# sidward14/gan-lab

Hardware: AMD Instinct MI355X
Metric: images/sec (G+D step), StyleGAN 1024^2 bs32/GPU (higher is better)
Workload: dtype f32; 1 GPU; StyleGAN res_samples=1024 FFHQ-shaped synthetic, bs=32/GPU fp32, nonsaturating + R1(lambda=10) + drift, stabilised phase, 1 D-iter + 1 G-iter; global_batch=32, per_gpu_batch=32, parallelism=single

## Files before the change

### gan_lab_amd/_lib.py

```python
import ctypes
import os
import subprocess

import torch

_HERE = os.path.dirname(os.path.abspath(__file__))
CSRC = os.path.join(_HERE, 'csrc')
SO_PATH = os.path.join(CSRC, os.path.basename(os.environ.get('GANLAB_HIP_LIB', '') or 'libganlab_hip.so'))

_c_int, _c_ll, _c_f, _c_p, _c_sz, _c_u64 = (ctypes.c_int, ctypes.c_longlong, ctypes.c_float, ctypes.c_void_p,
                                             ctypes.c_size_t, ctypes.c_uint64)

ACT_NONE, ACT_LRELU = 0, 1
PACK_FWD, PACK_DGRAD = 0, 1


class ConvGeom(ctypes.Structure):
    _fields_ = [('N', _c_int), ('Cin', _c_int), ('Hin', _c_int), ('Win', _c_int),
                ('Cout', _c_int), ('ks', _c_int), ('pad', _c_int), ('up', _c_int), ('pool', _c_int)]


_GP = ctypes.POINTER(ConvGeom)


# ... 41 lines not shown
    'ganlab_conv_splitk_plan': (_c_int, [_GP, _c_int]),
    'ganlab_conv_fwd_splitk_f32': (_c_int, [_c_p, _c_p, _c_p, _c_p, _GP, _c_f, _c_int, _c_f, _c_p, _c_sz, _c_p]),
    'ganlab_conv_dgrad_splitk_f32': (_c_int, [_c_p, _c_p, _c_p, _GP, _c_p, _c_sz, _c_p]),
    'ganlab_conv_dgrad_mask_supported': (_c_int, [_GP]),
    'ganlab_conv_dgrad_mask_f32': (_c_int, [_c_p, _c_p, _c_p, _c_p, _GP, _c_f, _c_p]),
    'ganlab_conv_act_bwd_fused_supported': (_c_int, [_GP]),
    'ganlab_conv_dgrad_act_f32': (_c_int, [_c_p, _c_p, _c_p, _c_p, _GP, _c_f, _c_p]),
    'ganlab_conv_fwd_mask_f32': (_c_int, [_c_p, _c_p, _c_p, _c_p, _GP, _c_f, _c_p]),
    'ganlab_conv_wgrad_act_f32': (_c_int, [_c_p, _c_p, _c_p, _c_p, _c_p, _GP, _c_f, _c_f, _c_f, _c_p, _c_sz, _c_p]),
    'ganlab_conv_wgrad_workspace': (_c_sz, [_GP]),
    'ganlab_conv_wgrad_f32': (_c_int, [_c_p, _c_p, _c_p, _GP, _c_f, _c_p, _c_sz, _c_p]),
    'ganlab_conv_s2_supported': (_c_int, [_GP]),
    'ganlab_conv_s2_pack_f32': (_c_ll, [_c_p, _c_p, _c_int, _c_int, _c_int, _c_int, _c_f, _c_p]),
    'ganlab_conv_s2_fwd_f32': (_c_int, [_c_p, _c_p, _c_p, _c_p, _GP, _c_f, _c_int, _c_f, _c_p]),
    'ganlab_conv_s2_dgrad_f32': (_c_int, [_c_p, _c_p, _c_p, _GP, _c_p]),
    'ganlab_conv_s2_wgrad_workspace': (_c_sz, [_GP]),
    'ganlab_conv_s2_wgrad_f32': (_c_int, [_c_p, _c_p, _c_p, _GP, _c_f, _c_p, _c_sz, _c_p]),
    'ganlab_conv_bf16_supported': (_c_int, [_GP]),
    'ganlab_conv_pack_bf16': (_c_ll, [_c_p, _c_p, _c_int, _c_int, _c_int, _c_f, _c_p]),
    'ganlab_conv_fwd_bf16': (_c_int, [_c_p, _c_p, _c_p, _c_p, _GP, _c_f, _c_int, _c_f, _c_p]),
    'ganlab_conv_dgrad_bf16': (_c_int, [_c_p, _c_p, _c_p, _GP, _c_p]),
    'ganlab_conv_bf16_splitk_plan': (_c_int, [_GP, _c_int]),
    'ganlab_conv_fwd_bf16_splitk': (_c_int, [_c_p, _c_p, _c_p, _c_p, _GP, _c_f, _c_int, _c_f, _c_p, _c_sz, _c_p]),
    'ganlab_conv_dgrad_bf16_splitk': (_c_int, [_c_p, _c_p, _c_p, _GP, _c_p, _c_sz, _c_p]),
    'ganlab_conv_wgrad_bf16_workspace': (_c_sz, [_GP]),
    'ganlab_conv_wgrad_bf16': (_c_int, [_c_p, _c_p, _c_p, _GP, _c_f, _c_p, _c_sz, _c_p]),
    'ganlab_conv_x3_supported': (_c_int, [_GP, _c_int]),
    'ganlab_conv_x3_pack': (_c_ll, [_c_p, _c_p, _c_int, _c_int, _c_int, _c_f, _c_p]),
    'ganlab_conv_fwd_x3': (_c_int, [_c_p, _c_p, _c_p, _c_p, _GP, _c_f, _c_int, _c_f, _c_p]),
    'ganlab_conv_dgrad_x3': (_c_int, [_c_p, _c_p, _c_p, _GP, _c_p]),
# ... 296 lines not shown
```

### gan_lab_amd/csrc/common.h

```cpp
#pragma once
#include <hip/hip_runtime.h>
#include <stdint.h>

#include "../../include/ganlab_hip.h"

typedef float f32x4 __attribute__((ext_vector_type(4)));

static thread_local int gl_launch_status = GANLAB_OK;
extern thread_local const void* gl_last_kernel_fn;
extern thread_local unsigned gl_last_grid;
#define GL_LAUNCH_RING 16
extern thread_local const void* gl_ring_fn[GL_LAUNCH_RING];
extern thread_local unsigned gl_ring_grid[GL_LAUNCH_RING];
extern thread_local unsigned long long gl_launch_count;
#define GL_LAUNCH(k, grid, ...)                                                  \
  do {                                                                           \
    (void)hipGetLastError();                                                     \
    const dim3 gl_grid_ = (grid);                                                \
    gl_last_kernel_fn = reinterpret_cast<const void*>(k);                        \
    gl_last_grid = gl_grid_.x * gl_grid_.y * gl_grid_.z;                         \
    gl_ring_fn[gl_launch_count % GL_LAUNCH_RING] = gl_last_kernel_fn;            \
    gl_ring_grid[gl_launch_count % GL_LAUNCH_RING] = gl_last_grid;               \
    ++gl_launch_count;                                                           \
    hipLaunchKernelGGL(k, gl_grid_, __VA_ARGS__);                                \
// ... 131 lines not shown
          const int kgq = ty * 2 + tx;
          base[((0 * 4 + kgq) * 128 + px * 64 + col) * 8 + j] = p.h;
          base[((1 * 4 + kgq) * 128 + px * 64 + col) * 8 + j] = p.m;
          base[((2 * 4 + kgq) * 128 + px * 64 + col) * 8 + j] = p.l;
        }
}

__device__ __forceinline__ float gl_comb_s2(int up, int a, int k) {
  if (up) {
    const int lo = (a == 0) ? 2 : (a == 1 ? 1 : 0), hi = (a == 0) ? 2 : (a == 1 ? 2 : (a == 2 ? 1 : 0));
    return (k >= lo && k <= hi) ? 1.f : 0.f;
  }
  const int lo = (a <= 1) ? 0 : (a == 2 ? 1 : 2), hi = (a == 0) ? 0 : (a == 1 ? 1 : 2);
  return (k >= lo && k <= hi) ? 0.5f : 0.f;
}
__device__ __forceinline__ void gl_x3_down_pack_position(const float* __restrict__ w9, int up, float scale, __bf16* __restrict__ out,
                                                         int CI, int ci, int co) {
  const int nsteps = CI / 8 * 4;
  const int ct = co >> 7, col = co & 127, q = ci >> 3, j = ci & 7;
  float k9[9];
#pragma unroll
  for (int t = 0; t < 9; ++t) k9[t] = w9[t];
#pragma unroll
  for (int a = 0; a < 4; ++a)
#pragma unroll
    for (int b = 0; b < 4; ++b) {
      float v = 0.f;
#pragma unroll
      for (int ky = 0; ky < 3; ++ky)
#pragma unroll
// ... 13 lines not shown

bool gl_wgrad_roll_supported(int N, int Cin, int Cout, int H, int W, int ks, int pad, int up, const void* x,
                             const void* gy);
int gl_wgrad_roll_slots(int N, int Cin, int Cout, int H, int W);
int gl_wgrad_roll_launch(const float* x, const float* gy, float* part, int N, int Cin, int Cout, int H, int W,
                         hipStream_t st, const float* aff_s = nullptr, const float* aff_t = nullptr);
bool gl_wgrad_s2_roll_supported(int N, int Cl, int Ch, int Hl, int Wl, const void* low, const void* high);
int gl_wgrad_s2_roll_slots(int N, int Cl, int Ch, int Hl, int Wl);
int gl_wgrad_s2_roll_launch(const float* low, const float* high, float* part, int N, int Cl, int Ch, int Hl, int Wl,
                            hipStream_t st, const float* aff_s = nullptr, const float* aff_t = nullptr);

bool gl_s2_roll_supported(int is_T, int N, int Cin, int Cout, int Hl, int Wl, const void* x, const void* y);
int gl_s2_roll_launch(int is_T, const float* x, const float* wp, const float* bias, float* y, int N, int Cin, int Cout,
                      int Hl, int Wl, int Cin_p, int Cout_p, float bias_scale, int act, float slope, hipStream_t st,
                      const float* aff_s = nullptr, const float* aff_t = nullptr);

bool gl_roll_blur_supported(int N, int Cin, int Cout, int H, int W, const void* x, const void* y);
int gl_roll_blur_launch(const float* x, const float* wp, const float* bias, float* y, void* bits, int N, int Cin, int Cout,
                        int H, int W, int Cin_p, int Cout_p, float bias_scale, float slope, hipStream_t st, int blur, int act);
```

### gan_lab_amd/csrc/conv_s2.hip

```cpp
#include "common.h"

#include <stdlib.h>

namespace {
typedef unsigned int u32x4 __attribute__((ext_vector_type(4)));

constexpr int round_up_c(int v, int m) { return (v + m - 1) / m * m; }
constexpr int ceil_div_c(int a, int b) { return (a + b - 1) / b; }
constexpr int pad_mod32(int v, int r) { return v + ((r - (v % 32)) + 32) % 32; }
inline int ceil_div(int a, int b) { return (a + b - 1) / b; }
inline bool aligned16(const void* p) { return (reinterpret_cast<uintptr_t>(p) & 15) == 0; }

__device__ __constant__ const int kDY[4] = {-1, 0, 0, 1};
__device__ __constant__ const int kPY[4] = {1, 0, 1, 0};
constexpr int cDY(int a) { return a == 0 ? -1 : (a == 3 ? 1 : 0); }
constexpr int cPY(int a) { return (a == 0 || a == 2) ? 1 : 0; }

__device__ __forceinline__ float comb(int up, int a, int k) {
  if (up) {
    const int lo = (a == 0) ? 2 : (a == 1 ? 1 : 0), hi = (a == 0) ? 2 : (a == 1 ? 2 : (a == 2 ? 1 : 0));
    return (k >= lo && k <= hi) ? 1.f : 0.f;
  }
  const int lo = (a <= 1) ? 0 : (a == 2 ? 1 : 2), hi = (a == 0) ? 0 : (a == 1 ? 1 : 2);
  return (k >= lo && k <= hi) ? 0.5f : 0.f;
// ... 5 lines not shown
  for (long long e = blockIdx.x * (long long)blockDim.x + threadIdx.x; e < total;
       e += (long long)gridDim.x * blockDim.x) {
    const int col = (int)(e % cols_p);
    const long long t = e / cols_p;
    const int row = (int)(t % rows_p), tap = (int)(t / rows_p);
    float v = 0.f;
    if (row < rows && col < cols) {
      const int co = transpose ? row : col, ci = transpose ? col : row;
      const int a = tap >> 2, b = tap & 3;
      const float* ws = w + ((long long)co * Cin + ci) * 9;
#pragma unroll
      for (int ky = 0; ky < 3; ++ky)
#pragma unroll
        for (int kx = 0; kx < 3; ++kx) v += comb(up, a, ky) * comb(up, b, kx) * ws[ky * 3 + kx];
      v *= scale;
    }
    out[e] = v;
  }
}

struct S2Args {
  const float* x;
  const float* wp;
  const float* bias;
  float* y;
  int N, Cin, Cout;
  int Hl, Wl;
  int Cin_p, Cout_p;
  int tiles_x, tiles_y, tiles_co;
  float bias_scale, slope;
// ... 1037 lines not shown
}

long long ganlab_conv_s2_pack_f32(const float* w, float* out, int Cout, int Cin, int up, int transpose, float scale,
                                  void* stream) {
  if (Cout <= 0 || Cin <= 0) return GANLAB_EINVAL;
  const int rows = transpose ? Cout : Cin, cols = transpose ? Cin : Cout;
  const int rows_p = round_up_c(rows, 16), cols_p = round_up_c(cols, 64);
  const long long total = 16LL * rows_p * cols_p;
  if (!out) return total;
  if (!w) return GANLAB_EINVAL;
  long long blocks = (total + 255) / 256;
  if (blocks > 4096) blocks = 4096;
  GL_LAUNCH(pack_s2_kernel, dim3((unsigned)blocks), dim3(256), 0, gl_stream(stream), w, out, Cout, Cin, rows, cols,
            rows_p, cols_p, up ? 1 : 0, transpose ? 1 : 0, scale);
  return GL_CHECK_LAUNCH() == GANLAB_OK ? total : GANLAB_ELAUNCH;
}

int ganlab_conv_s2_fwd_f32(const float* x, const float* wp, const float* bias, float* y, const ganlab_conv_geom* g,
                           float bias_scale, int act, float slope, void* stream) {
  int hl, wl;
  if (!s2_ok(g, &hl, &wl) || !x || !wp || !y || !aligned16(x) || !aligned16(wp) || !aligned16(y)) return GANLAB_EINVAL;
  S2Args a{};
  a.x = x; a.wp = wp; a.bias = bias; a.y = y;
  a.N = g->N; a.Cin = g->Cin; a.Cout = g->Cout; a.Hl = hl; a.Wl = wl;
  a.Cin_p = round_up_c(g->Cin, 16); a.Cout_p = round_up_c(g->Cout, 64);
  a.bias_scale = bias_scale; a.slope = slope; a.act = act;
  return g->pool ? run_S(a, gl_stream(stream)) : run_T(a, gl_stream(stream));
}

int ganlab_conv_s2_dgrad_f32(const float* gy, const float* wp, float* gx, const ganlab_conv_geom* g, void* stream) {
// ... 95 lines not shown
```

### gan_lab_amd/csrc/conv_s2_roll.hip

```cpp
#include "common.h"

#include <stdlib.h>

namespace {

typedef unsigned int u32x4 __attribute__((ext_vector_type(4)));
constexpr int SR_OOB = (int)0x80000000;

struct SRArgs {
  const float* x;
  const float* wp;
  const float* bias;
  float* y;
  int N, Cin, Cout;
  int Hl, Wl;
  int Cin_p, Cout_p;
  int cols, strips, spu;
  float bias_scale, slope;
  int act;
  const float* aff_s;
  const float* aff_t;
};

constexpr int SR_TW = 32;
// ... 127 lines not shown
#pragma unroll
      for (int r = 0; r < 4; ++r) {
        float v = (GL_ACC_DUMP ? acc[blk][r] + accb[blk][r] : acc[blk][r]) + bv;
        if (p.act == GANLAB_ACT_LRELU) v = gl_lrelu(v, p.slope);
        o[r] = __float_as_uint(v);
      }
      __builtin_amdgcn_raw_buffer_store_b128(o, rs_out, vo[blk] == SR_OOB ? vo[blk] : vo[blk] + orow, 0, 0);
      acc[blk] = f32x4{0.f, 0.f, 0.f, 0.f};
      accb[blk] = f32x4{0.f, 0.f, 0.f, 0.f};
    }
    __syncthreads();
    if constexpr (SR_SLOTS == 6) {
      store_rows(4 * t + 6, 4);
      __syncthreads();
    }
  }
}

constexpr int TR_TW = 32;
constexpr int TR_CP = 48;
constexpr int TR_SLOT = 32 * TR_CP;
constexpr int TR_SLOTS = 6;
constexpr int TR_Q = 10;
constexpr int TR_ITEMS = 2 * 32 * TR_Q;
constexpr int TR_PT = (TR_ITEMS + 255) / 256;

template <bool AFF>
__global__ __launch_bounds__(256, 3) void conv_s2_up_roll_kernel(SRArgs p) {
  __shared__ __attribute__((aligned(16))) float ring[TR_SLOTS * TR_SLOT];
  __shared__ float afftab[AFF ? 64 : 1];
// ... 175 lines not shown
                      int Hl, int Wl, int Cin_p, int Cout_p, float bias_scale, int act, float slope, hipStream_t st,
                      const float* aff_s, const float* aff_t) {
  if (aff_s != nullptr && !is_T) return GANLAB_EUNSUPPORTED;
  SRArgs a{};
  a.x = x; a.wp = wp; a.bias = bias; a.y = y; a.aff_s = aff_s; a.aff_t = aff_t;
  a.N = N; a.Cin = Cin; a.Cout = Cout; a.Hl = Hl; a.Wl = Wl; a.Cin_p = Cin_p; a.Cout_p = Cout_p;
  a.bias_scale = bias_scale; a.slope = slope; a.act = act;
  sr_plan(a, 4096);
  const long long grid = (long long)a.cols * a.strips * N;
  if (grid <= 0 || grid > 0x7fffffffLL) return GANLAB_EINVAL;
  if (is_T && aff_s != nullptr) GL_LAUNCH(conv_s2_up_roll_kernel<true>, dim3((unsigned)grid), dim3(256), 0, st, a);
  else if (is_T) GL_LAUNCH(conv_s2_up_roll_kernel<false>, dim3((unsigned)grid), dim3(256), 0, st, a);
  else GL_LAUNCH(conv_s2_down_roll_kernel, dim3((unsigned)grid), dim3(256), 0, st, a);
  return GL_CHECK_LAUNCH();
}
```

### gan_lab_amd/csrc/pack.hip

```cpp
#include "common.h"

namespace {

constexpr int round_up_c(int v, int m) { return (v + m - 1) / m * m; }

__global__ __launch_bounds__(256) void pack_many_kernel(const ganlab_pack_desc* __restrict__ descs, int n_desc) {
  int lo = 0, hi = n_desc - 1;
  const long long b = blockIdx.x;
  while (lo < hi) {
    const int mid = (lo + hi + 1) >> 1;
    if (descs[mid].block0 <= b) lo = mid; else hi = mid - 1;
  }
  const ganlab_pack_desc d = descs[lo];
  const long long e = (b - d.block0) * 256 + threadIdx.x;
  const float* w = d.src;
  if (d.kind == GANLAB_PACKKIND_PLAIN) {
    const int KK = d.ks * d.ks, dgrad = d.mode == GANLAB_PACK_DGRAD;
    const int rows = dgrad ? d.Cout : d.Cin, cols = dgrad ? d.Cin : d.Cout;
    const int rows_p = round_up_c(rows, d.ks == 1 ? 32 : 16), cols_p = round_up_c(cols, 64);
    const long long plane = (long long)rows_p * cols_p;
    if (e >= plane) return;
    const int col = (int)(e % cols_p), row = (int)(e / cols_p);
    const bool in = row < rows && col < cols;
    const int co = dgrad ? row : col, ci = dgrad ? col : row;
// ... 13 lines not shown
    float k9[9];
    const float* ws = w + ((long long)co * d.Cin + ci) * 9;
#pragma unroll
    for (int t = 0; t < 9; ++t) k9[t] = in ? ws[t] : 0.f;
    float* out = reinterpret_cast<float*>(d.dst) + e;
#pragma unroll
    for (int tap = 0; tap < 16; ++tap) {
      const int a = tap >> 2, bb = tap & 3;
      float v = 0.f;
#pragma unroll
      for (int ky = 0; ky < 3; ++ky)
#pragma unroll
        for (int kx = 0; kx < 3; ++kx) v += gl_comb_s2(d.up, a, ky) * gl_comb_s2(d.up, bb, kx) * k9[ky * 3 + kx];
      out[tap * plane] = v * d.scale;
    }
  } else if (d.kind == GANLAB_PACKKIND_X3 && d.ks == 4) {
    const int up = d.up;
    const int CO = up ? d.Cout : d.Cin, CI = up ? d.Cin : d.Cout;
    if (e >= (long long)CO * CI) return;
    int ci, co;
    if ((CO & 63) == 0) {
      const int col = (int)(e & 63);
      const long long t = e >> 6;
      ci = (int)(t % CI);
      co = (int)(t / CI) * 64 + col;
    } else {
      co = (int)(e % CO);
      ci = (int)(e / CO);
    }
    const float* w9 = up ? w + ((long long)co * d.Cin + ci) * 9 : w + ((long long)ci * d.Cin + co) * 9;
// ... 54 lines not shown
```

### gan_lab_amd/ops.py

```python
import ctypes
import os

import numpy as np

import torch
from torch.autograd import Function
from torch.autograd.function import once_differentiable

from . import _lib
from ._lib import ACT_LRELU, ACT_NONE, PACK_DGRAD, PACK_FWD, ConvGeom, check


def _p(t):
    return ctypes.c_void_p(t.data_ptr()) if t is not None else None


_RAW_STREAM = getattr(torch._C, '_cuda_getCurrentRawStream', None)
_GET_DEVICE = getattr(torch._C, '_cuda_getDevice', None)


def _st():
    if _RAW_STREAM is None or _GET_DEVICE is None:
        return ctypes.c_void_p(torch.cuda.current_stream().cuda_stream)
    return ctypes.c_void_p(_RAW_STREAM(_GET_DEVICE()))
# ... 119 lines not shown
    def out_shape(self):
        return (self.N, self.Cout, self.Ho, self.Wo)


def pool_fusable(N, Cin, Hin, Win, Cout, ks, pad):
    if ks != 3 or pad != 1:
        return False
    if _COMPUTE[0] == 'bf16':
        v = ConvGeom(int(N), int(Cin), int(Hin), int(Win), int(Cout), 3, 1, 0, 1)
        if _lib.lib().ganlab_conv_bf16_supported(ctypes.byref(v)):
            return True
    c = ConvGeom(int(N), int(Cin), int(Hin), int(Win), int(Cout), 3, 1, 0, 1)
    return bool(_lib.lib().ganlab_conv_s2_supported(ctypes.byref(c)))


class _PackEntry(object):
    __slots__ = ('w', 'out', 'serial', 'ptr', 'desc')


_PACK_CACHE = {}
_PACK_SERIAL = [0]
_PACK_GEN = [0]
_PACK_RANGES = {}
_PACK_TABLES = {}
_KIND_PLAIN, _KIND_S2, _KIND_BF16, _KIND_X3 = 0, 1, 2, 3


def bump_weight_epoch(ranges=None):
    _PACK_SERIAL[0] += 1
    if ranges is None:
        if _PACK_CACHE or _PACK_TABLES:
            _PACK_GEN[0] += 1
        _PACK_CACHE.clear()
        _PACK_TABLES.clear()
        _PACK_RANGES.clear()
        return
    for r in ranges:
        _PACK_RANGES[(int(r[0]), int(r[1]))] = _PACK_SERIAL[0]


# ... 4 lines not shown
_ALL_ADDRESSES = (0, 1 << 62)


def mark_packs_stale():
    if _PACK_RANGES:
        bump_weight_epoch(list(_PACK_RANGES.keys()))
    elif _PACK_CACHE:
        bump_weight_epoch([_ALL_ADDRESSES])


def _pack_one(e):
    L = _lib.lib()
    kind, cout, cin, ks, mode, up, scale, total = e.desc
    if kind == _KIND_S2:
        rc = L.ganlab_conv_s2_pack_f32(_p(e.w), _p(e.out), cout, cin, up, mode, scale, _st())
    elif kind == _KIND_BF16:
        rc = L.ganlab_conv_pack_bf16(_p(e.w), e.out.data_ptr(), cout, cin, mode, scale, _st())
    elif kind == _KIND_X3 and ks == 4:
        rc = L.ganlab_conv_s2_x3_pack(_p(e.w), e.out.data_ptr(), cout, cin, up, scale, _st())
    elif kind == _KIND_X3 and ks == 5:
        rc = L.ganlab_conv_s2_down_x3_pack(_p(e.w), e.out.data_ptr(), cout, cin, up, scale, _st())
    elif kind == _KIND_X3:
        rc = L.ganlab_conv_x3_pack(_p(e.w), e.out.data_ptr(), cout, cin, mode, scale, _st())
    else:
        rc = L.ganlab_conv_pack_f32(_p(e.w), _p(e.out), cout, cin, ks, mode, scale, _st())
    if rc != total:
        raise _lib.GanlabLibraryError(f're-pack failed ({rc} != {total})')


def _stale_range(e):
# ... 11 lines not shown
    tab = _PACK_TABLES.get(r)
    if (tab is None or tab[0] != keys) and torch.cuda.is_current_stream_capturing():
        for _, e in items:
            _pack_one(e)
            e.serial = _PACK_SERIAL[0]
        return
    if tab is None or tab[0] != keys:
        arr = (_lib.PackDesc * len(items))()
        blocks = 0
        for i, (_, e) in enumerate(items):
            kind, cout, cin, ks, mode, up, scale, total = e.desc
            d = arr[i]
            d.src, d.dst = e.w.data_ptr(), e.out.data_ptr()
            d.kind, d.Cout, d.Cin, d.ks, d.mode, d.up, d.scale, d.total, d.block0 = kind, cout, cin, ks, mode, up, scale, \
                total, blocks
            blocks += (total // (16 if kind == _KIND_S2 else (9 if kind == _KIND_BF16 else ((48 if ks >= 4 else 27) if kind == _KIND_X3 else ks * ks))) + 255) // 256
        host = torch.frombuffer(bytearray(bytes(arr)), dtype=torch.uint8)
        if tab is not None:
            _PACK_GEN[0] += 1
        tab = (keys, host.to(items[0][1].w.device), blocks)
        _PACK_TABLES[r] = tab
    check(L.ganlab_pack_many(tab[1].data_ptr(), len(items), tab[2], _st()), 'pack_many')
    now = _PACK_SERIAL[0]
    for _, e in items:
        e.serial = now


def _pack_lookup(key):
    e = _PACK_CACHE.get(key)
    if e is None:
        return None
    r = _stale_range(e)
    if r is not None:
        _repack_range(r)
    return e.out


def _pack_store(key, w, out, desc):
    if len(_PACK_CACHE) > 1024:
        bump_weight_epoch()
    e = _PackEntry()
    e.w, e.out, e.serial, e.ptr, e.desc = w.detach(), out, _PACK_SERIAL[0], w.data_ptr(), desc
    _PACK_CACHE[key] = e
    return out


def _packed(w, mode, scale, s2_up=None):
    key = (w.data_ptr(), w._version, tuple(w.shape), mode, float(scale), s2_up)
    hit = _pack_lookup(key)
    if hit is not None:
        return hit
    cout, cin, ks = w.shape[0], w.shape[1], w.shape[2]
    L = _lib.lib()
    if s2_up is not None:
        tr = 1 if mode == PACK_DGRAD else 0
        n = L.ganlab_conv_s2_pack_f32(None, None, cout, cin, int(s2_up), tr, scale, None)
        if n <= 0:
            raise _lib.GanlabLibraryError(f'conv_s2_pack size query failed ({n}) for weight {tuple(w.shape)}')
        out = _new((n,), w)
        rc = L.ganlab_conv_s2_pack_f32(_p(w), _p(out), cout, cin, int(s2_up), tr, scale, _st())
        if rc != n:
            raise _lib.GanlabLibraryError(f'conv_s2_pack failed ({rc})')
        return _pack_store(key, w, out, (_KIND_S2, cout, cin, 3, tr, int(s2_up), float(scale), int(n)))
    n = L.ganlab_conv_pack_f32(None, None, cout, cin, ks, mode, scale, None)
    if n <= 0:
        raise _lib.GanlabLibraryError(f'conv_pack size query failed ({n}) for weight {tuple(w.shape)}')
    out = _new((n,), w)
    rc = L.ganlab_conv_pack_f32(_p(w), _p(out), cout, cin, ks, mode, scale, _st())
    if rc != n:
        raise _lib.GanlabLibraryError(f'conv_pack failed ({rc})')
    return _pack_store(key, w, out, (_KIND_PLAIN, cout, cin, ks, mode, 0, float(scale), int(n)))


def _packed_bf16(w, mode, scale):
    key = (w.data_ptr(), w._version, tuple(w.shape), mode, float(scale), 'bf16')
    hit = _pack_lookup(key)
    if hit is not None:
        return hit
# ... 252 lines not shown
            ws = torch.empty((split * geom.N * geom.Cout * geom.Hin * m * geom.Win * m,), dtype=torch.float32, device=x.device)
            check(L.ganlab_conv_fwd_bf16_splitk(_p(xin), wp.data_ptr(), _p(bias), _p(y), ctypes.byref(geom), bias_scale, act,
                                                slope, _p(ws), ws.numel() * 4, _st()), 'conv_fwd_bf16_splitk')
            return y
        check(L.ganlab_conv_fwd_bf16(_p(xin), wp.data_ptr(), _p(bias), _p(y), ctypes.byref(geom), bias_scale,
                                     act, slope, _st()), 'conv_fwd_bf16')
        return y
    if x3_s2_down_ok(g):
        check(_lib.lib().ganlab_conv_s2_down_fwd_x3(_p(x), _packed_x3_s2_down(w, 0, scale).data_ptr(), _p(bias), _p(y), g.ref(),
                                                    bias_scale, act, slope, _st()), 'conv_s2_down_fwd_x3')
        return y
    if x3_s2_ok(g):
        check(_lib.lib().ganlab_conv_s2_fwd_x3(_p(x), _packed_x3_s2(w, 1, scale).data_ptr(), _p(bias), _p(y), g.ref(), bias_scale,
                                               act, slope, _st()), 'conv_s2_fwd_x3')
        return y
    if g.s2:
        wp = _packed(w, PACK_FWD, scale, s2_up=g.up)
        check(_lib.lib().ganlab_conv_s2_fwd_f32(_p(x), _p(wp), _p(bias), _p(y), g.ref(), bias_scale, act, slope,
                                                _st()), 'conv_s2_fwd')
        return y
    if g.ks == 1 and g.Hin == 1 and g.Win == 1 and g.N <= 64 and g.Cin >= 2048 and g.Cin % 128 == 0:
        g2 = Geom(1, g.Cout, g.Cin // 128, 128, g.N, 1, 0)
        obs = set_launch_observer(None)
        try:
            y = k_conv_wgrad(x.view(g2.out_shape), w.view(g2.in_shape), g2, scale).view(g.out_shape)
        finally:
            set_launch_observer(obs)
        if bias is not None or act != ACT_NONE:
            y = k_bias_act(y, bias, None, None, bias_scale, act, slope)
        return y
# ... 33 lines not shown
                check(L.ganlab_conv_dgrad_bf16(_p(gy), wp.data_ptr(), _p(out), ctypes.byref(geom), _st()), 'conv_dgrad_bf16')
            return out
        if g.bf_fused is not None:
            return run(g.bf_fused, _new(g.in_shape, gy))
        gxv = run(g.bf, _new((g.N, g.Cin, g.bf.Hin, g.bf.Win), gy))
        return k_pool2(gxv, 1.0) if g.up else gxv
    if x3_s2_down_ok(g, True):
        gx = _new(g.in_shape, gy)
        check(_lib.lib().ganlab_conv_s2_down_dgrad_x3(_p(gy), _packed_x3_s2_down(w, 1, scale).data_ptr(), _p(gx), g.ref(), _st()),
              'conv_s2_down_dgrad_x3')
        return gx
    if x3_s2_ok(g, True):
        gx = _new(g.in_shape, gy)
        check(_lib.lib().ganlab_conv_s2_dgrad_x3(_p(gy), _packed_x3_s2(w, 0, scale).data_ptr(), _p(gx), g.ref(), _st()),
              'conv_s2_dgrad_x3')
        return gx
    if g.s2:
        wp = _packed(w, PACK_DGRAD, scale, s2_up=g.up)
        gx = _new(g.in_shape, gy)
        check(_lib.lib().ganlab_conv_s2_dgrad_f32(_p(gy), _p(wp), _p(gx), g.ref(), _st()), 'conv_s2_dgrad')
        return gx
    if x3_ok(g, True):
        gx = _new(g.in_shape, gy)
        check(_lib.lib().ganlab_conv_dgrad_x3(_p(gy), _packed_x3(w, PACK_DGRAD, scale).data_ptr(), _p(gx), g.ref(), _st()),
              'conv_dgrad_x3')
        return gx
    wp = _packed(w, PACK_DGRAD, scale)
    hv, wv = (2 * g.Hin, 2 * g.Win) if g.up else (g.Hin, g.Win)
    gxv = _new((g.N, g.Cin, hv, wv), gy)
    split = 0 if g.up else _lib.lib().ganlab_conv_splitk_plan(g.ref(), 1)
# ... 3642 lines not shown
```

### include/ganlab_hip.h

```cpp
#ifndef GANLAB_HIP_H
#define GANLAB_HIP_H

#include <stddef.h>
#include <stdint.h>

#ifdef __cplusplus
extern "C" {
#endif

#define GANLAB_OK 0
#define GANLAB_EINVAL (-1)
#define GANLAB_EWORKSPACE (-2)
#define GANLAB_ELAUNCH (-3)
#define GANLAB_EUNSUPPORTED (-4)

#define GANLAB_ACT_NONE 0
#define GANLAB_ACT_LRELU 1

#define GANLAB_PACK_FWD 0
#define GANLAB_PACK_DGRAD 1

int ganlab_abi_version(void);

int ganlab_last_launch(char* name, int cap, unsigned* grid);
// ... 40 lines not shown
int ganlab_conv_wgrad_act_f32(const float* gy, const float* y, const float* x, float* gw, float* gb,
                              const ganlab_conv_geom* g, float scale, float bias_scale, float slope, void* workspace,
                              size_t workspace_bytes, void* stream);

size_t ganlab_conv_wgrad_workspace(const ganlab_conv_geom* g);
int ganlab_conv_wgrad_f32(const float* gy, const float* x, float* gw, const ganlab_conv_geom* g,
                          float scale, void* workspace, size_t workspace_bytes, void* stream);

int ganlab_conv_s2_supported(const ganlab_conv_geom* g);
long long ganlab_conv_s2_pack_f32(const float* w, float* out, int Cout, int Cin, int up, int transpose,
                                  float scale, void* stream);
int ganlab_conv_s2_fwd_f32(const float* x, const float* wp, const float* bias, float* y,
                           const ganlab_conv_geom* g, float bias_scale, int act, float slope, void* stream);
int ganlab_conv_s2_dgrad_f32(const float* gy, const float* wp, float* gx, const ganlab_conv_geom* g,
                             void* stream);
size_t ganlab_conv_s2_wgrad_workspace(const ganlab_conv_geom* g);
int ganlab_conv_s2_wgrad_f32(const float* gy, const float* x, float* gw, const ganlab_conv_geom* g,
                             float scale, void* workspace, size_t workspace_bytes, void* stream);

int ganlab_conv_bf16_supported(const ganlab_conv_geom* g);
long long ganlab_conv_pack_bf16(const float* w, void* out, int Cout, int Cin, int mode, float scale, void* stream);
int ganlab_conv_fwd_bf16(const float* x, const void* wp, const float* bias, float* y, const ganlab_conv_geom* g,
                         float bias_scale, int act, float slope, void* stream);
int ganlab_conv_dgrad_bf16(const float* gy, const void* wp, float* gx, const ganlab_conv_geom* g, void* stream);
int ganlab_conv_bf16_splitk_plan(const ganlab_conv_geom* g, int dgrad);
int ganlab_conv_fwd_bf16_splitk(const float* x, const void* wp, const float* bias, float* y, const ganlab_conv_geom* g,
                                float bias_scale, int act, float slope, void* workspace, size_t workspace_bytes,
                                void* stream);
int ganlab_conv_dgrad_bf16_splitk(const float* gy, const void* wp, float* gx, const ganlab_conv_geom* g, void* workspace,
                                  size_t workspace_bytes, void* stream);
// ... 270 lines not shown
int ganlab_conv_dgrad_rgb_sums_f32(const float* gy, const float* wp, const unsigned* ybits, const float* img, float* gw_rgb,
                                   float* gb_rgb, const ganlab_conv_geom* g, int img_c, float scale, float bias_scale,
                                   float slope, int acc_w, int acc_b, void* workspace, size_t workspace_bytes, void* stream);
int ganlab_conv_dgrad_act_bits_f32(const float* gy, const unsigned* ybits, const float* wp, float* gx,
                                   const ganlab_conv_geom* g, float slope, void* stream);
int ganlab_conv_fwd_mask_bits_f32(const float* x, const float* wp, const unsigned* ybits, float* out,
                                  const ganlab_conv_geom* g, float slope, void* stream);
int ganlab_conv_wgrad_act_bits_f32(const float* gy, const unsigned* ybits, const float* x, float* gw, float* gb,
                                   const ganlab_conv_geom* g, float scale, float bias_scale, float slope, void* workspace,
                                   size_t workspace_bytes, void* stream);

#define GANLAB_PACKKIND_PLAIN 0
#define GANLAB_PACKKIND_S2 1
#define GANLAB_PACKKIND_BF16 2
#define GANLAB_PACKKIND_X3 3
typedef struct ganlab_pack_desc {
  const float* src;
  void* dst;
  int kind;
  int Cout, Cin, ks;
  int mode;
  int up;
  float scale;
  int reserved;
  long long total;
  long long block0;
} ganlab_pack_desc;
int ganlab_pack_desc_size(void);
int ganlab_pack_many(const ganlab_pack_desc* descs_device, int n_desc, long long total_blocks, void* stream);

// ... 149 lines not shown
```

Baseline: 171.3 images/sec.

## Add box-filter stride-2 conv path that pre-sums 2x2 input before 3x3 MFMA

Adds a new stride-2 downsample (conv+2x2 avgpool) path that first sums 2x2 neighbourhoods of the full-resolution input into a shared-memory ring, then applies the plain 3x3 weights (scaled by 0.25) via MFMA. The existing path folds the pool into 4x4 combined weights. Reducing taps from 16 to 9 cuts MFMA work, and the same kernel also serves the dgrad of the upsample conv through flipped, transposed packing. It adds a new pack kind and more kernel complexity, and it only applies to small-channel geometries that gl_s2_roll_supported accepts.

```diff
diff --git a/gan_lab_amd/_lib.py b/gan_lab_amd/_lib.py
--- a/gan_lab_amd/_lib.py
+++ b/gan_lab_amd/_lib.py
@@ -79,6 +79,10 @@
     'ganlab_conv_s2_pack_f32': (_c_ll, [_c_p, _c_p, _c_int, _c_int, _c_int, _c_int, _c_f, _c_p]),
     'ganlab_conv_s2_fwd_f32': (_c_int, [_c_p, _c_p, _c_p, _c_p, _GP, _c_f, _c_int, _c_f, _c_p]),
     'ganlab_conv_s2_dgrad_f32': (_c_int, [_c_p, _c_p, _c_p, _GP, _c_p]),
+    'ganlab_conv_s2_box_supported': (_c_int, [_GP, _c_int]),
+    'ganlab_conv_s2_box_pack_f32': (_c_ll, [_c_p, _c_p, _c_int, _c_int, _c_int, _c_int, _c_f, _c_p]),
+    'ganlab_conv_s2_fwd_box_f32': (_c_int, [_c_p, _c_p, _c_p, _c_p, _GP, _c_f, _c_int, _c_f, _c_p]),
+    'ganlab_conv_s2_dgrad_box_f32': (_c_int, [_c_p, _c_p, _c_p, _GP, _c_p]),
     'ganlab_conv_s2_wgrad_workspace': (_c_sz, [_GP]),
     'ganlab_conv_s2_wgrad_f32': (_c_int, [_c_p, _c_p, _c_p, _GP, _c_f, _c_p, _c_sz, _c_p]),
     'ganlab_conv_bf16_supported': (_c_int, [_GP]),
diff --git a/gan_lab_amd/csrc/common.h b/gan_lab_amd/csrc/common.h
--- a/gan_lab_amd/csrc/common.h
+++ b/gan_lab_amd/csrc/common.h
@@ -169,6 +169,7 @@
   const int lo = (a <= 1) ? 0 : (a == 2 ? 1 : 2), hi = (a == 0) ? 0 : (a == 1 ? 1 : 2);
   return (k >= lo && k <= hi) ? 0.5f : 0.f;
 }
+__device__ __forceinline__ float gl_box_s2_factor(int up) { return up ? 1.f : 0.25f; }
 __device__ __forceinline__ void gl_x3_down_pack_position(const float* __restrict__ w9, int up, float scale, __bf16* __restrict__ out,
                                                          int CI, int ci, int co) {
   const int nsteps = CI / 8 * 4;
@@ -212,6 +213,8 @@
 int gl_s2_roll_launch(int is_T, const float* x, const float* wp, const float* bias, float* y, int N, int Cin, int Cout,
                       int Hl, int Wl, int Cin_p, int Cout_p, float bias_scale, int act, float slope, hipStream_t st,
                       const float* aff_s = nullptr, const float* aff_t = nullptr);
+int gl_s2_roll_box_launch(const float* x, const float* wp, const float* bias, float* y, int N, int Cin, int Cout, int Hl,
+                          int Wl, int Cin_p, int Cout_p, float bias_scale, int act, float slope, hipStream_t st);
 
 bool gl_roll_blur_supported(int N, int Cin, int Cout, int H, int W, const void* x, const void* y);
 int gl_roll_blur_launch(const float* x, const float* wp, const float* bias, float* y, void* bits, int N, int Cin, int Cout,
diff --git a/gan_lab_amd/csrc/conv_s2.hip b/gan_lab_amd/csrc/conv_s2.hip
--- a/gan_lab_amd/csrc/conv_s2.hip
+++ b/gan_lab_amd/csrc/conv_s2.hip
@@ -43,6 +43,23 @@
 #pragma unroll
         for (int kx = 0; kx < 3; ++kx) v += comb(up, a, ky) * comb(up, b, kx) * ws[ky * 3 + kx];
       v *= scale;
+    }
+    out[e] = v;
+  }
+}
+
+__global__ void pack_s2_box_kernel(const float* __restrict__ w, float* __restrict__ out, int Cout, int Cin, int rows,
+                                   int cols, int rows_p, int cols_p, int up, int transpose, float scale) {
+  const long long total = 9LL * rows_p * cols_p;
+  for (long long e = blockIdx.x * (long long)blockDim.x + threadIdx.x; e < total;
+       e += (long long)gridDim.x * blockDim.x) {
+    const int col = (int)(e % cols_p);
+    const long long t = e / cols_p;
+    const int row = (int)(t % rows_p), tap = (int)(t / rows_p);
+    float v = 0.f;
+    if (row < rows && col < cols) {
+      const int co = transpose ? row : col, ci = transpose ? col : row;
+      v = w[((long long)co * Cin + ci) * 9 + (up ? 8 - tap : tap)] * (scale * gl_box_s2_factor(up));
     }
     out[e] = v;
   }
@@ -1110,6 +1127,46 @@
   GL_LAUNCH(pack_s2_kernel, dim3((unsigned)blocks), dim3(256), 0, gl_stream(stream), w, out, Cout, Cin, rows, cols,
             rows_p, cols_p, up ? 1 : 0, transpose ? 1 : 0, scale);
   return GL_CHECK_LAUNCH() == GANLAB_OK ? total : GANLAB_ELAUNCH;
+}
+
+long long ganlab_conv_s2_box_pack_f32(const float* w, float* out, int Cout, int Cin, int up, int transpose, float scale,
+                                      void* stream) {
+  if (Cout <= 0 || Cin <= 0) return GANLAB_EINVAL;
+  const int rows = transpose ? Cout : Cin, cols = transpose ? Cin : Cout;
+  const int rows_p = round_up_c(rows, 16), cols_p = round_up_c(cols, 64);
+  const long long total = 9LL * rows_p * cols_p;
+  if (!out) return total;
+  if (!w) return GANLAB_EINVAL;
+  long long blocks = (total + 255) / 256;
+  if (blocks > 4096) blocks = 4096;
+  GL_LAUNCH(pack_s2_box_kernel, dim3((unsigned)blocks), dim3(256), 0, gl_stream(stream), w, out, Cout, Cin, rows, cols,
+            rows_p, cols_p, up ? 1 : 0, transpose ? 1 : 0, scale);
+  return GL_CHECK_LAUNCH() == GANLAB_OK ? total : GANLAB_ELAUNCH;
+}
+
+int ganlab_conv_s2_box_supported(const ganlab_conv_geom* g, int dgrad) {
+  int hl, wl;
+  if (!s2_ok(g, &hl, &wl)) return 0;
+  if (dgrad ? !g->up : !g->pool) return 0;
+  const int ci = dgrad ? g->Cout : g->Cin, co = dgrad ? g->Cin : g->Cout;
+  return gl_s2_roll_supported(0, g->N, ci, co, hl, wl, nullptr, nullptr) ? 1 : 0;
+}
+
+int ganlab_conv_s2_fwd_box_f32(const float* x, const float* wp, const float* bias, float* y, const ganlab_conv_geom* g,
+                               float bias_scale, int act, float slope, void* stream) {
+  int hl, wl;
+  if (!ganlab_conv_s2_box_supported(g, 0) || !s2_ok(g, &hl, &wl)) return GANLAB_EUNSUPPORTED;
+  if (!x || !wp || !y || !aligned16(x) || !aligned16(wp) || !aligned16(y)) return GANLAB_EINVAL;
+  return gl_s2_roll_box_launch(x, wp, bias, y, g->N, g->Cin, g->Cout, hl, wl, round_up_c(g->Cin, 16),
+                               round_up_c(g->Cout, 64), bias_scale, act, slope, gl_stream(stream));
+}
+
+int ganlab_conv_s2_dgrad_box_f32(const float* gy, const float* wp, float* gx, const ganlab_conv_geom* g, void* stream) {
+  int hl, wl;
+  if (!ganlab_conv_s2_box_supported(g, 1) || !s2_ok(g, &hl, &wl)) return GANLAB_EUNSUPPORTED;
+  if (!gy || !wp || !gx || !aligned16(gy) || !aligned16(wp) || !aligned16(gx)) return GANLAB_EINVAL;
+  return gl_s2_roll_box_launch(gy, wp, nullptr, gx, g->N, g->Cout, g->Cin, hl, wl, round_up_c(g->Cout, 16),
+                               round_up_c(g->Cin, 64), 0.f, GANLAB_ACT_NONE, 0.f, gl_stream(stream));
 }
 
 int ganlab_conv_s2_fwd_f32(const float* x, const float* wp, const float* bias, float* y, const ganlab_conv_geom* g,
diff --git a/gan_lab_amd/csrc/conv_s2_roll.hip b/gan_lab_amd/csrc/conv_s2_roll.hip
--- a/gan_lab_amd/csrc/conv_s2_roll.hip
+++ b/gan_lab_amd/csrc/conv_s2_roll.hip
@@ -165,6 +165,155 @@
       store_rows(4 * t + 6, 4);
       __syncthreads();
     }
+  }
+}
+
+constexpr int SB_SLOTS = 9;
+
+__global__ __launch_bounds__(256, 3) void conv_s2_down_roll_box_kernel(SRArgs p) {
+  __shared__ __attribute__((aligned(16))) float ring[SB_SLOTS * SR_SLOT];
+  constexpr int NG = 12, PD = 2;
+  const int tid = threadIdx.x, lane = tid & 63, wv = tid >> 6;
+  const int mco = wv & 1, jrow = wv >> 1;
+  const int px = lane & 15, kk = lane >> 4;
+  int bid = gl_xcd_remap(blockIdx.x, gridDim.x);
+  const int col = bid % p.cols;
+  bid /= p.cols;
+  const int strip = bid % p.strips;
+  const int n = bid / p.strips;
+  const int X0 = col * SR_TW, Ys = strip * p.spu * 2;
+  const int nsteps = min(p.spu, p.Hl / 2 - strip * p.spu);
+  const int H = 2 * p.Hl, W = 2 * p.Wl, hplane = H * W;
+  const long long lplane = (long long)p.Hl * p.Wl;
+
+  const int sci = tid >> 4, sq = tid & 15;
+  const int gmain = sci < p.Cin ? (sci * hplane + 2 * X0 + 4 * sq) * 4 : SR_OOB;
+  const int lmain = sci * SR_CP + 2 * sq;
+  const bool halo = tid < 128;
+  const int hci = tid & 15, hk = (tid >> 4) & 3, hside = (tid >> 6) & 1;
+  const int hc0 = hside ? 2 * X0 + 63 : 2 * X0 - 1;
+  const int hg0 = (halo && hci < p.Cin && hc0 >= 0) ? (hci * hplane + hc0) * 4 : SR_OOB;
+  const int hg1 = (halo && hci < p.Cin && hc0 + 1 < W) ? (hci * hplane + hc0 + 1) * 4 : SR_OOB;
+  const int lhalo = hci * SR_CP + 41 + 32 * hside;
+
+  float wreg[36];
+#pragma unroll
+  for (int i = 0; i < 36; ++i)
+    wreg[i] = p.wp[(long long)((i >> 2) * p.Cin_p + (i & 3) * 4 + kk) * p.Cout_p + mco * 16 + px];
+  const int co = mco * 16 + px;
+  const bool co_ok = co < p.Cout;
+  const float bv = (p.bias != nullptr && co_ok) ? p.bias[co] * p.bias_scale : 0.f;
+
+  const __amdgpu_buffer_rsrc_t rs_in = __builtin_amdgcn_make_buffer_rsrc(
+      const_cast<float*>(p.x + (long long)n * p.Cin * hplane), 0, (unsigned)(p.Cin * hplane * 4), 0x00020000);
+  const __amdgpu_buffer_rsrc_t rs_out = __builtin_amdgcn_make_buffer_rsrc(
+      p.y + (long long)n * p.Cout * lplane, 0, (unsigned)(p.Cout * lplane * 4), 0x00020000);
+  int vo[2];
+#pragma unroll
+  for (int blk = 0; blk < 2; ++blk)
+    vo[blk] = co_ok ? (int)(((long long)co * lplane + X0 + blk * 16 + 4 * kk) * 4) : SR_OOB;
+
+  float4 xr[4];
+  float hx[4];
+  float4 carry = float4{0.f, 0.f, 0.f, 0.f};
+  auto load_block = [&](int b0, int nb) {
+#pragma unroll
+    for (int k = 0; k < 4; ++k) {
+      const int vy = 2 * Ys + b0 + k;
+      const bool ok = gmain != SR_OOB && k < nb && (unsigned)vy < (unsigned)H;
+      const u32x4 v = __builtin_amdgcn_raw_buffer_load_b128(rs_in, ok ? gmain + (int)((unsigned)vy * (unsigned)(W * 4)) : SR_OOB, 0, 0);
+      xr[k] = float4{__uint_as_float(v.x), __uint_as_float(v.y), __uint_as_float(v.z), __uint_as_float(v.w)};
+    }
+#pragma unroll
+    for (int j = 0; j < 2; ++j) {
+      const int vy = 2 * Ys - 1 + b0 + hk + j;
+      const bool ok = hk < nb && (unsigned)vy < (unsigned)H;
+      const int ro = (int)((unsigned)vy * (unsigned)(W * 4));
+      hx[2 * j] = __uint_as_float(__builtin_amdgcn_raw_buffer_load_b32(rs_in, (ok && hg0 != SR_OOB) ? hg0 + ro : SR_OOB, 0, 0));
+      hx[2 * j + 1] = __uint_as_float(__builtin_amdgcn_raw_buffer_load_b32(rs_in, (ok && hg1 != SR_OOB) ? hg1 + ro : SR_OOB, 0, 0));
+    }
+  };
+  auto hsum = [&](const float4 v) {
+    const float nx = __builtin_bit_cast(float, __builtin_amdgcn_update_dpp(0, __builtin_bit_cast(int, v.x), 0x101, 0xf, 0xf, true));
+    return float4{v.x + v.y, v.y + v.z, v.z + v.w, v.w + nx};
+  };
+  auto store_block = [&](int b0, int nb) {
+#pragma unroll
+    for (int k = 0; k < 4; ++k) {
+      const float4 h = hsum(xr[k]);
+      if (k < nb) {
+        float* d = ring + ((b0 + k) % SB_SLOTS) * SR_SLOT + lmain;
+        *reinterpret_cast<float2*>(d) = float2{carry.x + h.x, carry.z + h.z};
+        if (sq < 15) *reinterpret_cast<float2*>(d + 42) = float2{carry.y + h.y, carry.w + h.w};
+        else d[42] = carry.y + h.y;
+        carry = h;
+      }
+    }
+    if (halo && hk < nb) ring[((b0 + hk) % SB_SLOTS) * SR_SLOT + lhalo] = (hx[0] + hx[1]) + (hx[2] + hx[3]);
+  };
+
+  f32x4 acc[2] = {f32x4{0.f, 0.f, 0.f, 0.f}, f32x4{0.f, 0.f, 0.f, 0.f}};
+  [[maybe_unused]] f32x4 accb[2] = {f32x4{0.f, 0.f, 0.f, 0.f}, f32x4{0.f, 0.f, 0.f, 0.f}};
+  load_block(-1, 1);
+  carry = hsum(xr[0]);
+  load_block(0, 4);
+  store_block(0, 4);
+  load_block(4, 1);
+  store_block(4, 1);
+  __syncthreads();
+  const int lane_off = kk * SR_CP + px;
+  for (int t = 0; t < nsteps; ++t) {
+    int sb[3];
+#pragma unroll
+    for (int a = 0; a < 3; ++a) sb[a] = ((4 * t + 2 * jrow + a) % SB_SLOTS) * SR_SLOT + lane_off;
+    float rb[PD + 1][2][3];
+    auto fetch = [&](int g, int s) {
+      const int a = g >> 2, c4 = g & 3;
+      const float* src = ring + sb[a] + c4 * 4 * SR_CP;
+#pragma unroll
+      for (int blk = 0; blk < 2; ++blk) {
+        rb[s][blk][0] = src[blk * 16];
+        rb[s][blk][1] = src[blk * 16 + 41];
+        rb[s][blk][2] = src[blk * 16 + 42];
+      }
+    };
+#pragma unroll
+    for (int g = 0; g < PD; ++g) fetch(g, g % (PD + 1));
+#pragma unroll
+    for (int g = 0; g < NG; ++g) {
+      if (g + PD < NG) fetch(g + PD, (g + PD) % (PD + 1));
+      const int s = g % (PD + 1), a = g >> 2, c4 = g & 3;
+#pragma unroll
+      for (int b = 0; b < 3; ++b) {
+        const int v = b == 0 ? 1 : (b == 1 ? 0 : 2);
+#pragma unroll
+        for (int blk = 0; blk < 2; ++blk) {
+          if (GL_ACC_DUMP && g >= NG / 2)
+            accb[blk] = __builtin_amdgcn_mfma_f32_16x16x4f32(rb[s][blk][v], wreg[(a * 3 + b) * 4 + c4], accb[blk], 0, 0, 0);
+          else
+            acc[blk] = __builtin_amdgcn_mfma_f32_16x16x4f32(rb[s][blk][v], wreg[(a * 3 + b) * 4 + c4], acc[blk], 0, 0, 0);
+        }
+      }
+      if (g == 1) load_block(4 * t + 5, t + 1 < nsteps ? 4 : 0);
+      __builtin_amdgcn_sched_barrier(0);
+    }
+    store_block(4 * t + 5, 4);
+    const int Y = Ys + 2 * t + jrow;
+    const int orow = Y * p.Wl * 4;
+#pragma unroll
+    for (int blk = 0; blk < 2; ++blk) {
+      u32x4 o;
+#pragma unroll
+      for (int r = 0; r < 4; ++r) {
+        float v = (GL_ACC_DUMP ? acc[blk][r] + accb[blk][r] : acc[blk][r]) + bv;
+        if (p.act == GANLAB_ACT_LRELU) v = gl_lrelu(v, p.slope);
+        o[r] = __float_as_uint(v);
+      }
+      __builtin_amdgcn_raw_buffer_store_b128(o, rs_out, vo[blk] == SR_OOB ? vo[blk] : vo[blk] + orow, 0, 0);
+      acc[blk] = f32x4{0.f, 0.f, 0.f, 0.f};
+      accb[blk] = f32x4{0.f, 0.f, 0.f, 0.f};
+    }
+    __syncthreads();
   }
 }
 
@@ -370,3 +519,16 @@
   else GL_LAUNCH(conv_s2_down_roll_kernel, dim3((unsigned)grid), dim3(256), 0, st, a);
   return GL_CHECK_LAUNCH();
 }
+
+int gl_s2_roll_box_launch(const float* x, const float* wp, const float* bias, float* y, int N, int Cin, int Cout, int Hl,
+                          int Wl, int Cin_p, int Cout_p, float bias_scale, int act, float slope, hipStream_t st) {
+  SRArgs a{};
+  a.x = x; a.wp = wp; a.bias = bias; a.y = y;
+  a.N = N; a.Cin = Cin; a.Cout = Cout; a.Hl = Hl; a.Wl = Wl; a.Cin_p = Cin_p; a.Cout_p = Cout_p;
+  a.bias_scale = bias_scale; a.slope = slope; a.act = act;
+  sr_plan(a, 4096);
+  const long long grid = (long long)a.cols * a.strips * N;
+  if (grid <= 0 || grid > 0x7fffffffLL) return GANLAB_EINVAL;
+  GL_LAUNCH(conv_s2_down_roll_box_kernel, dim3((unsigned)grid), dim3(256), 0, st, a);
+  return GL_CHECK_LAUNCH();
+}
diff --git a/gan_lab_amd/csrc/pack.hip b/gan_lab_amd/csrc/pack.hip
--- a/gan_lab_amd/csrc/pack.hip
+++ b/gan_lab_amd/csrc/pack.hip
@@ -51,6 +51,20 @@
         for (int kx = 0; kx < 3; ++kx) v += gl_comb_s2(d.up, a, ky) * gl_comb_s2(d.up, bb, kx) * k9[ky * 3 + kx];
       out[tap * plane] = v * d.scale;
     }
+  } else if (d.kind == GANLAB_PACKKIND_S2BOX) {
+    const int transpose = d.mode;
+    const int rows = transpose ? d.Cout : d.Cin, cols = transpose ? d.Cin : d.Cout;
+    const int rows_p = round_up_c(rows, 16), cols_p = round_up_c(cols, 64);
+    const long long plane = (long long)rows_p * cols_p;
+    if (e >= plane) return;
+    const int col = (int)(e % cols_p), row = (int)(e / cols_p);
+    const bool in = row < rows && col < cols;
+    const int co = transpose ? row : col, ci = transpose ? col : row;
+    const float* ws = w + ((long long)co * d.Cin + ci) * 9;
+    float* out = reinterpret_cast<float*>(d.dst) + e;
+#pragma unroll
+    for (int tap = 0; tap < 9; ++tap)
+      out[tap * plane] = in ? ws[d.up ? 8 - tap : tap] * (d.scale * gl_box_s2_factor(d.up)) : 0.f;
   } else if (d.kind == GANLAB_PACKKIND_X3 && d.ks == 4) {
     const int up = d.up;
     const int CO = up ? d.Cout : d.Cin, CI = up ? d.Cin : d.Cout;
diff --git a/gan_lab_amd/ops.py b/gan_lab_amd/ops.py
--- a/gan_lab_amd/ops.py
+++ b/gan_lab_amd/ops.py
@@ -157,6 +157,12 @@
     return bool(_lib.lib().ganlab_conv_s2_supported(ctypes.byref(c)))
 
 
+def s2_box_ok(g, dgrad):
+    if os.environ.get('GANLAB_S2_BOX') == '0':
+        return False
+    return bool(_lib.lib().ganlab_conv_s2_box_supported(g.ref(), 1 if dgrad else 0))
+
+
 class _PackEntry(object):
     __slots__ = ('w', 'out', 'serial', 'ptr', 'desc')
 
@@ -166,7 +172,7 @@
 _PACK_GEN = [0]
 _PACK_RANGES = {}
 _PACK_TABLES = {}
-_KIND_PLAIN, _KIND_S2, _KIND_BF16, _KIND_X3 = 0, 1, 2, 3
+_KIND_PLAIN, _KIND_S2, _KIND_BF16, _KIND_X3, _KIND_S2BOX = 0, 1, 2, 3, 4
 
 
 def bump_weight_epoch(ranges=None):
@@ -201,6 +207,8 @@
     kind, cout, cin, ks, mode, up, scale, total = e.desc
     if kind == _KIND_S2:
         rc = L.ganlab_conv_s2_pack_f32(_p(e.w), _p(e.out), cout, cin, up, mode, scale, _st())
+    elif kind == _KIND_S2BOX:
+        rc = L.ganlab_conv_s2_box_pack_f32(_p(e.w), _p(e.out), cout, cin, up, mode, scale, _st())
     elif kind == _KIND_BF16:
         rc = L.ganlab_conv_pack_bf16(_p(e.w), e.out.data_ptr(), cout, cin, mode, scale, _st())
     elif kind == _KIND_X3 and ks == 4:
@@ -242,7 +250,7 @@
             d.src, d.dst = e.w.data_ptr(), e.out.data_ptr()
             d.kind, d.Cout, d.Cin, d.ks, d.mode, d.up, d.scale, d.total, d.block0 = kind, cout, cin, ks, mode, up, scale, \
                 total, blocks
-            blocks += (total // (16 if kind == _KIND_S2 else (9 if kind == _KIND_BF16 else ((48 if ks >= 4 else 27) if kind == _KIND_X3 else ks * ks))) + 255) // 256
+            blocks += (total // (16 if kind == _KIND_S2 else (9 if kind in (_KIND_BF16, _KIND_S2BOX) else ((48 if ks >= 4 else 27) if kind == _KIND_X3 else ks * ks))) + 255) // 256
         host = torch.frombuffer(bytearray(bytes(arr)), dtype=torch.uint8)
         if tab is not None:
             _PACK_GEN[0] += 1
@@ -273,8 +281,8 @@
     return out
 
 
-def _packed(w, mode, scale, s2_up=None):
-    key = (w.data_ptr(), w._version, tuple(w.shape), mode, float(scale), s2_up)
+def _packed(w, mode, scale, s2_up=None, box=False):
+    key = (w.data_ptr(), w._version, tuple(w.shape), mode, float(scale), s2_up) + (('box',) if box else ())
     hit = _pack_lookup(key)
     if hit is not None:
         return hit
@@ -282,14 +290,15 @@
     L = _lib.lib()
     if s2_up is not None:
         tr = 1 if mode == PACK_DGRAD else 0
-        n = L.ganlab_conv_s2_pack_f32(None, None, cout, cin, int(s2_up), tr, scale, None)
+        pack = L.ganlab_conv_s2_box_pack_f32 if box else L.ganlab_conv_s2_pack_f32
+        n = pack(None, None, cout, cin, int(s2_up), tr, scale, None)
         if n <= 0:
             raise _lib.GanlabLibraryError(f'conv_s2_pack size query failed ({n}) for weight {tuple(w.shape)}')
         out = _new((n,), w)
-        rc = L.ganlab_conv_s2_pack_f32(_p(w), _p(out), cout, cin, int(s2_up), tr, scale, _st())
+        rc = pack(_p(w), _p(out), cout, cin, int(s2_up), tr, scale, _st())
         if rc != n:
             raise _lib.GanlabLibraryError(f'conv_s2_pack failed ({rc})')
-        return _pack_store(key, w, out, (_KIND_S2, cout, cin, 3, tr, int(s2_up), float(scale), int(n)))
+        return _pack_store(key, w, out, (_KIND_S2BOX if box else _KIND_S2, cout, cin, 3, tr, int(s2_up), float(scale), int(n)))
     n = L.ganlab_conv_pack_f32(None, None, cout, cin, ks, mode, scale, None)
     if n <= 0:
         raise _lib.GanlabLibraryError(f'conv_pack size query failed ({n}) for weight {tuple(w.shape)}')
@@ -572,6 +581,11 @@
         check(_lib.lib().ganlab_conv_s2_fwd_x3(_p(x), _packed_x3_s2(w, 1, scale).data_ptr(), _p(bias), _p(y), g.ref(), bias_scale,
                                                act, slope, _st()), 'conv_s2_fwd_x3')
         return y
+    if g.s2 and s2_box_ok(g, False):
+        wp = _packed(w, PACK_FWD, scale, s2_up=g.up, box=True)
+        check(_lib.lib().ganlab_conv_s2_fwd_box_f32(_p(x), _p(wp), _p(bias), _p(y), g.ref(), bias_scale, act, slope,
+                                                    _st()), 'conv_s2_fwd_box')
+        return y
     if g.s2:
         wp = _packed(w, PACK_FWD, scale, s2_up=g.up)
         check(_lib.lib().ganlab_conv_s2_fwd_f32(_p(x), _p(wp), _p(bias), _p(y), g.ref(), bias_scale, act, slope,
@@ -635,6 +649,11 @@
         gx = _new(g.in_shape, gy)
         check(_lib.lib().ganlab_conv_s2_dgrad_x3(_p(gy), _packed_x3_s2(w, 0, scale).data_ptr(), _p(gx), g.ref(), _st()),
               'conv_s2_dgrad_x3')
+        return gx
+    if g.s2 and s2_box_ok(g, True):
+        wp = _packed(w, PACK_DGRAD, scale, s2_up=g.up, box=True)
+        gx = _new(g.in_shape, gy)
+        check(_lib.lib().ganlab_conv_s2_dgrad_box_f32(_p(gy), _p(wp), _p(gx), g.ref(), _st()), 'conv_s2_dgrad_box')
         return gx
     if g.s2:
         wp = _packed(w, PACK_DGRAD, scale, s2_up=g.up)
diff --git a/include/ganlab_hip.h b/include/ganlab_hip.h
--- a/include/ganlab_hip.h
+++ b/include/ganlab_hip.h
@@ -78,6 +78,13 @@
                            const ganlab_conv_geom* g, float bias_scale, int act, float slope, void* stream);
 int ganlab_conv_s2_dgrad_f32(const float* gy, const float* wp, float* gx, const ganlab_conv_geom* g,
                              void* stream);
+int ganlab_conv_s2_box_supported(const ganlab_conv_geom* g, int dgrad);
+long long ganlab_conv_s2_box_pack_f32(const float* w, float* out, int Cout, int Cin, int up, int transpose,
+                                      float scale, void* stream);
+int ganlab_conv_s2_fwd_box_f32(const float* x, const float* wp, const float* bias, float* y,
+                               const ganlab_conv_geom* g, float bias_scale, int act, float slope, void* stream);
+int ganlab_conv_s2_dgrad_box_f32(const float* gy, const float* wp, float* gx, const ganlab_conv_geom* g,
+                                 void* stream);
 size_t ganlab_conv_s2_wgrad_workspace(const ganlab_conv_geom* g);
 int ganlab_conv_s2_wgrad_f32(const float* gy, const float* x, float* gw, const ganlab_conv_geom* g,
                              float scale, void* workspace, size_t workspace_bytes, void* stream);
@@ -378,6 +385,7 @@
 #define GANLAB_PACKKIND_S2 1
 #define GANLAB_PACKKIND_BF16 2
 #define GANLAB_PACKKIND_X3 3
+#define GANLAB_PACKKIND_S2BOX 4
 typedef struct ganlab_pack_desc {
   const float* src;
   void* dst;
```

Result: no change. 171.3 images/sec, median of 2 (+0.0%).
